# bwittmann/transoar

Measured on AMD Instinct MI355X. Metric: training-step CT volumes/s, 160x160x256 Focused-Decoder, higher is better.
Workload: dtype bf16

## Files before the change

include/transoar_convgemm.h:

```cpp
#ifndef TRANSOAR_CONVGEMM_H
#define TRANSOAR_CONVGEMM_H

#ifdef __cplusplus
extern "C" {
#endif

enum {
  TRANSOAR_CONVGEMM_OK = 0,
  TRANSOAR_CONVGEMM_ERR_NULL = -1,
  TRANSOAR_CONVGEMM_ERR_DIM = -2
};

int transoar_conv3d_igemm(const void* x, const void* wk, const float* bias, void* y, float* y32,
                          int N, int SD, int SH, int SW, int Cin, int Cout,
                          int MD, int MH, int MW, int src_stride,
                          int OD, int OH, int OW, int out_stride, int opd, int oph, int opw,
                          unsigned taps_d, unsigned taps_h, unsigned taps_w, int split, int classes, void* hip_stream);

int transoar_conv3d_finish(const float* y32, const float* bias, void* y, long rows, int cout, int split, void* hip_stream);

int transoar_conv3d_dgrad_s2_halo(const void* dy, const void* wkt, void* dx, int N, int OD, int OH, int OW, int D, int H, int W,
                                  int Cin, int Cout, void* hip_stream);

long transoar_conv3d_wgrad_part_floats(int Cin, int Cout, int chunks, int taps_out);
int transoar_conv3d_wgrad(const void* dy, const void* x, float* part, float* dw, int N, int SD, int SH, int SW, int Cin,
                          int Cout, int MD, int MH, int MW, int src_stride,
                          unsigned taps_d, unsigned taps_h, unsigned taps_w, int chunks, int taps_out, void* hip_stream);

int transoar_linear_wgrad_bias(const void* dy, const void* x, float* part, float* dw, float* bias_part, float* db, int T, int Cin,
                               int Cout, int chunks, void* hip_stream);

int transoar_conv3d_wgrad_ring(const void* dy, const void* x, float* part, float* dw, int N, int SD, int SH, int SW, int Cin,
                               int Cout, int MD, int MH, int MW, int src_stride, int chunks, void* hip_stream);

int transoar_conv3d_pack(const float* w, void* wk, void* wkt, int Cout, int Cin, void* hip_stream);

int transoar_conv3d_pack_many(const void* table, int n_layers, long total_tiles, void* hip_stream);

int transoar_convgemm_abi_version(void);

#ifdef __cplusplus
}
#endif
#endif
```

transoar_amd/conv_gemm.py:

```python
import ctypes
import os

import torch

from . import _native

_PKG = os.path.dirname(os.path.abspath(__file__))
_LIB_PATH = os.path.join(_PKG, "libtransoar_convgemm.so")
ABI_VERSION = 3
CL3D = torch.channels_last_3d


def _load():
    if not os.path.exists(_LIB_PATH):
        raise _native.NativeLibraryError("%s is not built (python transoar_amd/_build.py)" % _LIB_PATH)
    lib = ctypes.CDLL(_LIB_PATH)
    i, p, u = ctypes.c_int, ctypes.c_void_p, ctypes.c_uint
    lib.transoar_conv3d_igemm.restype = i
    lib.transoar_conv3d_igemm.argtypes = [p] * 5 + [i] * 17 + [u] * 3 + [i, i, p]
    lib.transoar_conv3d_finish.restype = i
    lib.transoar_conv3d_finish.argtypes = [p, p, p, ctypes.c_long, i, i, p]
    lib.transoar_conv3d_wgrad.restype = i
    lib.transoar_conv3d_wgrad.argtypes = [p, p, p, p] + [i] * 10 + [u] * 3 + [i, i, p]
    lib.transoar_linear_wgrad_bias.restype = i
    lib.transoar_linear_wgrad_bias.argtypes = [p] * 6 + [i] * 4 + [p]
    lib.transoar_conv3d_wgrad_ring.restype = i
    lib.transoar_conv3d_wgrad_ring.argtypes = [p, p, p, p] + [i] * 11 + [p]
    lib.transoar_conv3d_wgrad_part_floats.restype = ctypes.c_long
    lib.transoar_conv3d_wgrad_part_floats.argtypes = [i, i, i, i]
    lib.transoar_conv3d_dgrad_s2_halo.restype = i
    lib.transoar_conv3d_dgrad_s2_halo.argtypes = [p, p, p] + [i] * 9 + [p]
    lib.transoar_conv3d_pack.restype = i
    lib.transoar_conv3d_pack.argtypes = [p, p, p, i, i, p]
    lib.transoar_conv3d_pack_many.restype = i
    lib.transoar_conv3d_pack_many.argtypes = [p, i, ctypes.c_long, p]
    lib.transoar_convgemm_abi_version.restype = i
    if lib.transoar_convgemm_abi_version() != ABI_VERSION:
        raise _native.NativeLibraryError("%s: ABI mismatch, rebuild" % _LIB_PATH)
    return lib


lib = _load()


def _taps(entries):
    v = len(entries)
    for e, (delta, t) in enumerate(entries):
        v |= ((delta + 1) << (2 + 4 * e)) | (t << (4 + 4 * e))
    return v


TAPS_FWD = _taps([(-1, 0), (0, 1), (1, 2)])
TAPS_DGRAD1 = _taps([(1, 0), (0, 1), (-1, 2)])
TAPS_PARITY = (_taps([(0, 1)]), _taps([(1, 0), (0, 2)]))
TAPS_ONE = _taps([(0, 1)])

SPLIT_BELOW_TILES = 384
DGRAD_S2_HALO = os.environ.get("TRANSOAR_DGRAD_S2_HALO", "1") != "0"
WGRAD_BLOCKS = 512


def _check(rc, what):
    if rc != 0:
        raise RuntimeError("%s failed with code %d" % (what, rc))


def _stream():
    return torch.cuda.current_stream().cuda_stream


def pack_fwd(weight):
    co, ci = weight.shape[:2]
    return weight.permute(2, 3, 4, 0, 1).reshape(27, co, ci).to(torch.bfloat16).contiguous()


def pack_dgrad(weight):
    co, ci = weight.shape[:2]
    return weight.permute(2, 3, 4, 1, 0).reshape(27, ci, co).to(torch.bfloat16).contiguous()


def pack_both(weight):
    co, ci = weight.shape[:2]
    if weight.dtype != torch.float32 or not weight.is_contiguous() or not os.environ.get("TRANSOAR_CONV_PACK_HIP"):
        return pack_fwd(weight), pack_dgrad(weight)
    wk = torch.empty((27, co, ci), dtype=torch.bfloat16, device=weight.device)
    wkt = torch.empty((27, ci, co), dtype=torch.bfloat16, device=weight.device)
    with torch.cuda.device(weight.device):
        _check(lib.transoar_conv3d_pack(weight.data_ptr(), wk.data_ptr(), wkt.data_ptr(), co, ci, _stream()), "transoar_conv3d_pack")
    return wk, wkt


class PackPlan:

    def __init__(self, modules):
        self.modules = list(modules)
        assert self.modules
        dev = self.modules[0].weight.device
        self.buffers, rows, tile = [], [], 0
        for m in self.modules:
            w = m.weight
            assert w.dtype == torch.float32 and w.is_contiguous() and tuple(w.shape[2:]) == (3, 3, 3) and w.device == dev
            co, ci = w.shape[:2]
            wk = torch.empty((27, co, ci), dtype=torch.bfloat16, device=dev)
            wkt = torch.empty((27, ci, co), dtype=torch.bfloat16, device=dev)
            self.buffers.append((wk, wkt))
            rows.append([w.data_ptr(), wk.data_ptr(), wkt.data_ptr(), co | (ci << 32), tile])
            tile += ((co + 31) // 32) * ((ci + 31) // 32)
        self.total_tiles = tile
        self.ptrs = [r[0] for r in rows]
        self.table = torch.tensor(rows, dtype=torch.int64, device=dev)

    def valid(self):
        return all(m.weight.data_ptr() == p for m, p in zip(self.modules, self.ptrs))

    def run(self):
        with torch.cuda.device(self.table.device):
            _check(lib.transoar_conv3d_pack_many(self.table.data_ptr(), len(self.modules), self.total_tiles, _stream()),
                   "transoar_conv3d_pack_many")
        for m, packs in zip(self.modules, self.buffers):
            m._packs, m._packs_version = packs, m.weight._version


def _split_for(tiles, k_steps):
    if tiles >= SPLIT_BELOW_TILES:
        return 1
    return max(1, min((SPLIT_BELOW_TILES + tiles - 1) // tiles, k_steps // 4, 16))


def _tiles(rows, cout):
    bn = 64 if cout <= 64 else 128
    return ((rows + 127) // 128) * ((cout + bn - 1) // bn)


def _igemm(x, wk, bias, out, src_dims, cin, cout, m_dims, src_stride, out_dims, out_stride, parity, taps, n, split, classes=0):
    b = bias.data_ptr() if bias is not None else None
    with torch.cuda.device(x.device):
        if split > 1:
            rows_out = n * out_dims[0] * out_dims[1] * out_dims[2]
            part = torch.empty((split, rows_out, cout), dtype=torch.float32, device=x.device)
            _check(lib.transoar_conv3d_igemm(x.data_ptr(), wk.data_ptr(), None, None, part.data_ptr(), n, *src_dims, cin, cout,
                                             *m_dims, src_stride, *out_dims, out_stride, *parity, *taps, split, classes, _stream()),
                   "transoar_conv3d_igemm")
            _check(lib.transoar_conv3d_finish(part.data_ptr(), b, out.data_ptr(), rows_out, cout, split, _stream()),
                   "transoar_conv3d_finish")
        else:
            _check(lib.transoar_conv3d_igemm(x.data_ptr(), wk.data_ptr(), b, out.data_ptr(), None, n, *src_dims, cin, cout,
                                             *m_dims, src_stride, *out_dims, out_stride, *parity, *taps, 1, classes, _stream()),
                   "transoar_conv3d_igemm")


MAX_ROWS = 1 << 21


def _batch_chunks(n, rows_per_sample, what):
    if n * rows_per_sample < MAX_ROWS:
        return [(0, n)]
    per = (MAX_ROWS - 1) // rows_per_sample
    if per < 1:
        raise RuntimeError("%s: one sample has %d rows, the implicit-GEMM kernels address < %d per launch"
                           % (what, rows_per_sample, MAX_ROWS))
    return [(i, min(per, n - i)) for i in range(0, n, per)]


def conv_forward(x, wk, bias, stride, split=None):
    n, ci, d, h, w = x.shape
    co = wk.shape[1]
    od, oh, ow = (d - 1) // stride + 1, (h - 1) // stride + 1, (w - 1) // stride + 1
    chunks = _batch_chunks(n, od * oh * ow, "conv_forward")
    if len(chunks) > 1:
        y = torch.empty((n, co, od, oh, ow), dtype=torch.bfloat16, device=x.device, memory_format=CL3D)
        for i, c in chunks:
            y[i:i + c] = conv_forward(x[i:i + c], wk, bias, stride, split)
        return y
    y = torch.empty((n, co, od, oh, ow), dtype=torch.bfloat16, device=x.device, memory_format=CL3D)
    if split is None:
        split = _split_for(_tiles(n * od * oh * ow, co), (27 * ci + 63) // 64)
    _igemm(x, wk, bias, y, (d, h, w), ci, co, (od, oh, ow), stride, (od, oh, ow), 1, (0, 0, 0), (TAPS_FWD,) * 3, n, split)
    return y


def conv_dgrad(gy, wkt, stride, in_dims, split=None):
    n, co, od, oh, ow = gy.shape
    ci = wkt.shape[1]
    d, h, w = in_dims
    gx = torch.empty((n, ci, d, h, w), dtype=torch.bfloat16, device=gy.device, memory_format=CL3D)
    halo = split is None and stride == 2 and DGRAD_S2_HALO and ci <= 32 and co in (16, 32, 48)
    chunks = [(0, n)] if halo else _batch_chunks(n, d * h * w, "conv_dgrad")
    if len(chunks) > 1:
        for i, c in chunks:
            gx[i:i + c] = conv_dgrad(gy[i:i + c], wkt, stride, in_dims, split)
        return gx
    if stride == 1:
        if split is None:
            split = _split_for(_tiles(n * d * h * w, ci), (27 * co + 63) // 64)
        _igemm(gy, wkt, None, gx, (od, oh, ow), co, ci, (d, h, w), 1, (d, h, w), 1, (0, 0, 0), (TAPS_DGRAD1,) * 3, n, split)
        return gx
    if split is None and DGRAD_S2_HALO and ci <= 32 and co in (16, 32, 48):
        with torch.cuda.device(gy.device):
            _check(lib.transoar_conv3d_dgrad_s2_halo(gy.data_ptr(), wkt.data_ptr(), gx.data_ptr(), n, od, oh, ow, d, h, w, ci, co, _stream()),
                   "transoar_conv3d_dgrad_s2_halo")
        return gx
    if split is None:
        split = _split_for(_tiles(n * d * h * w, ci), (8 * co + 63) // 64)
    _igemm(gy, wkt, None, gx, (od, oh, ow), co, ci, (1, 1, 1), 1, (d, h, w), 2, (0, 0, 0), (TAPS_ONE,) * 3, n, split, classes=1)
    return gx


def _wgrad(x2, gy2, geom, taps, taps_out, out_shape):
    n, sd, sh, sw, ci, co, md, mh, mw, stride = geom
    nt = 1
    for t in taps:
        nt *= t & 3
    bt = 64 if (ci <= 64 and co <= 64) else 128
    tiles = nt * ((co + bt - 1) // bt) * ((ci + bt - 1) // bt)
    rows = n * md * mh * mw
    budget = WGRAD_BLOCKS * (2 if (rows >= (1 << 20) or tiles >= 64) else 1)
    chunks = max(1, min(budget // tiles, rows // 1024 if rows >= 1024 else 1))
    part = torch.empty(lib.transoar_conv3d_wgrad_part_floats(ci, co, chunks, taps_out), dtype=torch.float32, device=x2.device)
    dw = torch.empty(out_shape, dtype=torch.float32, device=x2.device)
    with torch.cuda.device(x2.device):
        _check(lib.transoar_conv3d_wgrad(gy2.data_ptr(), x2.data_ptr(), part.data_ptr(), dw.data_ptr(), n, sd, sh, sw, ci, co, md, mh, mw,
                                         stride, *taps, chunks, taps_out, _stream()), "transoar_conv3d_wgrad")
    return dw


WGRAD_RING = os.environ.get("TRANSOAR_WGRAD_RING", "1") != "0"
WGRAD_RING_CHUNKS = 85


def wgrad_ring_supported(ci, co, ow, rows):
    return (WGRAD_RING and ci <= 64 and co <= 64 and max(ci, co) > 32 and ci % 8 == 0 and co % 8 == 0 and ow % 64 == 0
            and rows >= (1 << 18))


def conv_wgrad_ring(x, gy, stride, chunks=None):
    n, ci, d, h, w = x.shape
    co, od, oh, ow = gy.shape[1:]
    chunks = chunks or WGRAD_RING_CHUNKS
    part = torch.empty(lib.transoar_conv3d_wgrad_part_floats(ci, co, chunks, 27), dtype=torch.float32, device=x.device)
    dw = torch.empty((co, ci, 3, 3, 3), dtype=torch.float32, device=x.device)
    with torch.cuda.device(x.device):
        _check(lib.transoar_conv3d_wgrad_ring(gy.data_ptr(), x.data_ptr(), part.data_ptr(), dw.data_ptr(), n, d, h, w, ci, co, od, oh, ow,
                                              stride, chunks, _stream()), "transoar_conv3d_wgrad_ring")
    return dw


def conv_wgrad(x, gy, stride):
    n, ci, d, h, w = x.shape
    co, od, oh, ow = gy.shape[1:]
    if wgrad_ring_supported(ci, co, ow, n * od * oh * ow):
        return conv_wgrad_ring(x, gy, stride)
    chunks = _batch_chunks(n, od * oh * ow, "conv_wgrad")
    if len(chunks) > 1:
        dw = None
        for i, c in chunks:
            part = conv_wgrad(x[i:i + c], gy[i:i + c], stride)
            dw = part if dw is None else dw.add_(part)
        return dw
    return _wgrad(x, gy, (n, d, h, w, ci, co, od, oh, ow, stride), (TAPS_FWD,) * 3, 27, (co, ci, 3, 3, 3))


def linear_wgrad(x, gy):
    t, k = x.shape
    nn_ = gy.shape[1]
    return _wgrad(x, gy, (1, 1, 1, t, k, nn_, 1, 1, t, 1), (TAPS_ONE,) * 3, 1, (nn_, k))


def linear_wgrad_bias_usable(k, n):
    return k % (64 if (k <= 64 and n <= 64) else 128) != 0


def linear_wgrad_bias(x, gy):
    t, k = x.shape
    nn_ = gy.shape[1]
    bt = 64 if (k <= 64 and nn_ <= 64) else 128
    tiles = ((nn_ + bt - 1) // bt) * ((k + bt - 1) // bt)
    budget = WGRAD_BLOCKS * (2 if (t >= (1 << 20) or tiles >= 64) else 1)
    chunks = max(1, min(budget // tiles, t // 1024 if t >= 1024 else 1))
    part = torch.empty(lib.transoar_conv3d_wgrad_part_floats(k, nn_, chunks, 1), dtype=torch.float32, device=x.device)
    bias_part = torch.empty(chunks * nn_, dtype=torch.float32, device=x.device)
    dw = torch.empty((nn_, k), dtype=torch.float32, device=x.device)
    db = torch.empty(nn_, dtype=torch.float32, device=x.device)
    with torch.cuda.device(x.device):
        _check(lib.transoar_linear_wgrad_bias(gy.data_ptr(), x.data_ptr(), part.data_ptr(), dw.data_ptr(), bias_part.data_ptr(), db.data_ptr(),
                                              t, k, nn_, chunks, _stream()), "transoar_linear_wgrad_bias")
    return dw, db


def supported(cin, cout, rows):
    return cin % 8 == 0 and cout % 8 == 0 and cin >= 8 and rows < (1 << 21)
```

transoar_amd/csrc/conv_gemm.hip:

```cpp
#include <hip/hip_runtime.h>
#include <stdint.h>

#include "../../include/transoar_convgemm.h"

namespace {

typedef float f32x16 __attribute__((ext_vector_type(16)));
typedef short s16x8 __attribute__((ext_vector_type(8)));
typedef short s16x4 __attribute__((ext_vector_type(4)));
typedef __bf16 bf16x8_t __attribute__((ext_vector_type(8)));
typedef unsigned int u32x4 __attribute__((ext_vector_type(4)));

constexpr int BM = 128, BK = 64;
constexpr int kTile = BM * BK * 2;

__device__ __forceinline__ f32x16 mfma(s16x8 a, s16x8 b, f32x16 c) {
  return __builtin_amdgcn_mfma_f32_32x32x16_bf16(__builtin_bit_cast(bf16x8_t, a), __builtin_bit_cast(bf16x8_t, b), c, 0, 0, 0);
}
__device__ __forceinline__ unsigned short f32_to_bf16(float f) {
  return __builtin_bit_cast(unsigned short, static_cast<__bf16>(f));
}
typedef __attribute__((address_space(3))) void conv_lds_void;
__device__ __forceinline__ void dma16(__amdgpu_buffer_rsrc_t rs, unsigned voff, unsigned dst) {
  unsigned keep;
// ... 278 lines not shown
    for (int e = 0; e < 8; ++e) v[e] += bias[c + e];
  }
  u32x4 o;
#pragma unroll
  for (int e = 0; e < 4; ++e) o[e] = static_cast<unsigned>(f32_to_bf16(v[2 * e])) | (static_cast<unsigned>(f32_to_bf16(v[2 * e + 1])) << 16);
  reinterpret_cast<u32x4*>(y)[i] = o;
}

constexpr int WK = 64;
constexpr int kSegRows = 2048;

template <int TW>
__global__ __launch_bounds__(256, 2) void conv3d_wgrad_kernel(
    const unsigned short* __restrict__ DY, const unsigned short* __restrict__ X, float* __restrict__ part, ConvGeom g,
    unsigned tp_d, unsigned tp_h, unsigned tp_w, int chunks, int rows_per_chunk, int tiles_co, int tiles_ci, int slabs,
    unsigned dy_bytes, unsigned x_bytes, float* __restrict__ bias_part) {
  constexpr int BT = 64 * TW;
  constexpr int WP = 2 * BT;
  constexpr int PR = 8 * TW;
  __shared__ __attribute__((aligned(16))) unsigned char lds[2][2 * WK * WP];
  __shared__ unsigned xrow[kSegRows];
  const int tid = threadIdx.x, lane = tid & 63, wave = tid >> 6;
  const int wm = wave >> 1, wn = wave & 1;
  const int nd = taps_count(tp_d), nh = taps_count(tp_h), nw = taps_count(tp_w);
  const int ntaps = nd * nh * nw;
  long bid = xcd_contiguous(blockIdx.x, static_cast<long>(chunks) * tiles_ci * tiles_co * ntaps);
  if (bid < 0) return;
  const int tci = static_cast<int>(bid % tiles_ci); bid /= tiles_ci;
  const int tco = static_cast<int>(bid % tiles_co); bid /= tiles_co;
  const int tap = static_cast<int>(bid % ntaps); bid /= ntaps;
  const int chunk = static_cast<int>(bid);
  const int ed = tap / (nh * nw), r_ = tap - ed * nh * nw, eh = r_ / nw, ew = r_ - eh * nw;
  const int dd = taps_delta(tp_d, ed), dh = taps_delta(tp_h, eh), dw = taps_delta(tp_w, ew);
  const int slab = (taps_t(tp_d, ed) * 3 + taps_t(tp_h, eh)) * 3 + taps_t(tp_w, ew);
  const int M = g.N * g.MD * g.MH * g.MW;
  const int m_beg = chunk * rows_per_chunk, m_end = min(M, m_beg + rows_per_chunk);
  const int co0 = tco * BT, ci0 = tci * BT;
  const __amdgpu_buffer_rsrc_t rdy = __builtin_amdgcn_make_buffer_rsrc(const_cast<unsigned short*>(DY), 0, static_cast<int>(dy_bytes), 0x00020000);
  const __amdgpu_buffer_rsrc_t rx = __builtin_amdgcn_make_buffer_rsrc(const_cast<unsigned short*>(X), 0, static_cast<int>(x_bytes), 0x00020000);

  constexpr int NS = WK * PR / 256, RS = 256 / PR;
  const int s_piece = tid % PR, s_row = tid / PR;
  auto row_swz = [](int r) -> int { return TW == 2 ? (r & 3) << 2 : ((r >> 1) & 1) << 2; };
  const int l_piece = s_piece ^ row_swz(s_row);
  const bool co_ok = co0 + l_piece * 8 < g.Cout, ci_ok = ci0 + l_piece * 8 < g.Cin;
  const unsigned y_col = co_ok ? static_cast<unsigned>(co0 + l_piece * 8) * 2u : 0x80000000u;
  const unsigned x_col = ci_ok ? static_cast<unsigned>(ci0 + l_piece * 8) * 2u : 0x80000000u;
  const bool bias_here = bias_part != nullptr && tci == tiles_ci - 1;
  const bool ones_piece = bias_here && ci0 + l_piece * 8 == g.Cin;
  if (ones_piece) {
#pragma unroll
    for (int st = 0; st < 2; ++st)
#pragma unroll
      for (int i = 0; i < WK * PR / 256; ++i)
        *reinterpret_cast<u32x4*>(&lds[st][WK * WP + (s_row + (256 / PR) * i) * WP + s_piece * 16]) = u32x4{0x00003f80u, 0u, 0u, 0u};
  }
  const float inv_mw = 1.0f / static_cast<float>(g.MW), inv_mh = 1.0f / static_cast<float>(g.MH), inv_md = 1.0f / static_cast<float>(g.MD);
  auto fill_rows = [&](int seg_beg, int seg_end) {
    for (int m = seg_beg + tid; m < seg_end; m += 256) {
      const int r1 = static_cast<int>((static_cast<float>(m) + 0.5f) * inv_mw), mw = m - r1 * g.MW;
      const int r2 = static_cast<int>((static_cast<float>(r1) + 0.5f) * inv_mh), mh = r1 - r2 * g.MH;
      const int nb = static_cast<int>((static_cast<float>(r2) + 0.5f) * inv_md), md = r2 - nb * g.MD;
      const int sd = md * g.src_stride + dd, sh = mh * g.src_stride + dh, sw = mw * g.src_stride + dw;
      const bool ok = static_cast<unsigned>(sd) < static_cast<unsigned>(g.SD) && static_cast<unsigned>(sh) < static_cast<unsigned>(g.SH) &&
                      static_cast<unsigned>(sw) < static_cast<unsigned>(g.SW);
      xrow[m - seg_beg] = ok ? static_cast<unsigned>(((nb * g.SD + sd) * g.SH + sh) * g.SW + sw) * static_cast<unsigned>(g.Cin) * 2u : 0x80000000u;
    }
  };
  int seg0 = 0, seg1 = 0;
  const unsigned lds0 = static_cast<unsigned>(reinterpret_cast<size_t>((conv_lds_void*)&lds[0][0]));
  const unsigned dst0 = __builtin_amdgcn_readfirstlane(lds0 + static_cast<unsigned>(wave) * 1024u);
  auto dma_step = [&](int m_base, int stage) {
    const unsigned base = dst0 + static_cast<unsigned>(stage) * (2u * WK * WP);
#pragma unroll
    for (int i = 0; i < NS; ++i) {
      const int m = m_base + s_row + RS * i;
      const bool in = m < seg1;
      const unsigned xo = in ? xrow[m - seg0] : 0x80000000u;
      dma16(rdy, in ? static_cast<unsigned>(m) * static_cast<unsigned>(g.Cout) * 2u + y_col : 0x80000000u, base + i * (RS * WP));
      if (!ones_piece) dma16(rx, xo + x_col, base + WK * WP + i * (RS * WP));
    }
  };
  f32x16 acc[TW][TW];
#pragma unroll
  for (int a = 0; a < TW; ++a)
#pragma unroll
    for (int b = 0; b < TW; ++b)
#pragma unroll
      for (int i = 0; i < 16; ++i) acc[a][b][i] = 0.f;
  const int kg = lane >> 5;
  const int t_row = 8 * kg + ((lane & 15) >> 2), t_ch = 16 * ((lane >> 4) & 1) + 4 * (lane & 3);
  typedef __attribute__((address_space(3))) s16x4 lds_s16x4;
  const int t_swz = row_swz(t_row) * 16;
  auto frag = [&](const unsigned char* tile, int k16, int ch0) -> s16x8 {
    const unsigned char* p = tile + (k16 * 16 + t_row) * WP + (((ch0 + t_ch) * 2) ^ t_swz);
    const s16x4 lo = __builtin_amdgcn_ds_read_tr16_b64_v4i16((lds_s16x4*)(p));
    const s16x4 hi = __builtin_amdgcn_ds_read_tr16_b64_v4i16((lds_s16x4*)(p + 4 * WP));
    return __builtin_shufflevector(lo, hi, 0, 1, 2, 3, 4, 5, 6, 7);
  };
  auto compute = [&](int stage) {
    const unsigned char* ty = lds[stage];
    const unsigned char* tx = lds[stage] + WK * WP;
#pragma unroll
    for (int k16 = 0; k16 < WK / 16; ++k16) {
      s16x8 fy[TW], fx[TW];
#pragma unroll
      for (int i = 0; i < TW; ++i) {
        fy[i] = frag(ty, k16, wm * 32 * TW + i * 32);
        fx[i] = frag(tx, k16, wn * 32 * TW + i * 32);
      }
#pragma unroll
      for (int a = 0; a < TW; ++a)
#pragma unroll
        for (int b = 0; b < TW; ++b) acc[a][b] = mfma(fy[a], fx[b], acc[a][b]);
    }
  };
  for (seg0 = m_beg; seg0 < m_end; seg0 += kSegRows) {
    seg1 = min(m_end, seg0 + kSegRows);
    __syncthreads();
    fill_rows(seg0, seg1);
    __syncthreads();
    const int steps = (seg1 - seg0 + WK - 1) / WK;
    dma_step(seg0, 0);
    dma_wait();
    block_barrier();
    for (int s = 0; s < steps; s += 2) {
      if (s + 1 < steps) dma_step(seg0 + (s + 1) * WK, 1);
      compute(0);
      dma_wait();
      block_barrier();
      if (s + 1 >= steps) break;
      if (s + 2 < steps) dma_step(seg0 + (s + 2) * WK, 0);
      compute(1);
      dma_wait();
      block_barrier();
    }
  }
  float* dst = part + (static_cast<long>(chunk) * slabs + (slabs == 1 ? 0 : slab)) * g.Cout * g.Cin;
#pragma unroll
  for (int a = 0; a < TW; ++a)
#pragma unroll
    for (int b = 0; b < TW; ++b) {
      const int ci = ci0 + wn * 32 * TW + b * 32 + (lane & 31);
      if (bias_here && ci == g.Cin) {
#pragma unroll
        for (int r = 0; r < 16; ++r) {
          const int co = co0 + wm * 32 * TW + a * 32 + (r & 3) + 8 * (r >> 2) + 4 * kg;
          if (co < g.Cout) bias_part[static_cast<long>(chunk) * g.Cout + co] = acc[a][b][r];
        }
      }
      if (ci >= g.Cin) continue;
#pragma unroll
      for (int r = 0; r < 16; ++r) {
        const int co = co0 + wm * 32 * TW + a * 32 + (r & 3) + 8 * (r >> 2) + 4 * kg;
        if (co < g.Cout) dst[static_cast<long>(co) * g.Cin + ci] = acc[a][b][r];
      }
    }
}

constexpr int kReducePairs = 128;
__global__ __launch_bounds__(256) void conv3d_wgrad_reduce_kernel(const float* __restrict__ part, float* __restrict__ dw, int chunks,
                                                                  int slabs, long coci) {
  __shared__ __attribute__((aligned(16))) float sh[kReducePairs * 27];
  const long e0 = static_cast<long>(blockIdx.x) * kReducePairs;
  const int quads = kReducePairs / 4;
  const int work = quads * slabs;
  if (work < 256) {
    const int P = 256 / work;
    const int sub = threadIdx.x / work, idx = threadIdx.x - sub * work;
    const int tap = idx / quads, q = idx - tap * quads;
    float4 v{0.f, 0.f, 0.f, 0.f};
    if (sub < P && e0 + 4 * q < coci) {
      const float* src = part + static_cast<long>(tap) * coci + e0 + 4 * q;
      const long step = static_cast<long>(slabs) * coci;
      int k = sub;
      for (; k + 3 * P < chunks; k += 4 * P) {
        const float4 a = *reinterpret_cast<const float4*>(src + (k + 0 * P) * step), b = *reinterpret_cast<const float4*>(src + (k + 1 * P) * step);
        const float4 c = *reinterpret_cast<const float4*>(src + (k + 2 * P) * step), d = *reinterpret_cast<const float4*>(src + (k + 3 * P) * step);
        v.x += (a.x + b.x) + (c.x + d.x); v.y += (a.y + b.y) + (c.y + d.y);
        v.z += (a.z + b.z) + (c.z + d.z); v.w += (a.w + b.w) + (c.w + d.w);
      }
      for (; k < chunks; k += P) {
        const float4 a = *reinterpret_cast<const float4*>(src + k * step);
        v.x += a.x; v.y += a.y; v.z += a.z; v.w += a.w;
      }
    }
    float4* turn = reinterpret_cast<float4*>(sh);
    if (sub < P) turn[sub * work + idx] = v;
    __syncthreads();
    if (sub == 0) {
      for (int g2 = 1; g2 < P; ++g2) {
        const float4 o = turn[g2 * work + idx];
        v.x += o.x; v.y += o.y; v.z += o.z; v.w += o.w;
      }
    }
    __syncthreads();
    if (sub == 0) {
      sh[(4 * q + 0) * slabs + tap] = v.x;
      sh[(4 * q + 1) * slabs + tap] = v.y;
      sh[(4 * q + 2) * slabs + tap] = v.z;
      sh[(4 * q + 3) * slabs + tap] = v.w;
    }
  } else {
  for (int idx = threadIdx.x; idx < quads * slabs; idx += 256) {
    const int tap = idx / quads, q = idx - tap * quads;
    float4 v{0.f, 0.f, 0.f, 0.f};
    if (e0 + 4 * q < coci) {
      const float* src = part + static_cast<long>(tap) * coci + e0 + 4 * q;
      const long step = static_cast<long>(slabs) * coci;
      int k = 0;
      for (; k + 4 <= chunks; k += 4) {
        const float4 a = *reinterpret_cast<const float4*>(src + (k + 0) * step), b = *reinterpret_cast<const float4*>(src + (k + 1) * step);
        const float4 c = *reinterpret_cast<const float4*>(src + (k + 2) * step), d = *reinterpret_cast<const float4*>(src + (k + 3) * step);
        v.x += (a.x + b.x) + (c.x + d.x); v.y += (a.y + b.y) + (c.y + d.y);
        v.z += (a.z + b.z) + (c.z + d.z); v.w += (a.w + b.w) + (c.w + d.w);
      }
      for (; k < chunks; ++k) {
        const float4 a = *reinterpret_cast<const float4*>(src + k * step);
        v.x += a.x; v.y += a.y; v.z += a.z; v.w += a.w;
      }
    }
    sh[(4 * q + 0) * slabs + tap] = v.x;
    sh[(4 * q + 1) * slabs + tap] = v.y;
    sh[(4 * q + 2) * slabs + tap] = v.z;
    sh[(4 * q + 3) * slabs + tap] = v.w;
  }
  }
  __syncthreads();
  const long total = coci * slabs, base = e0 * slabs;
  for (int idx = threadIdx.x; idx < quads * slabs; idx += 256)
    if (base + 4 * idx < total) *reinterpret_cast<float4*>(dw + base + 4 * idx) = *reinterpret_cast<const float4*>(&sh[4 * idx]);
}

__global__ __launch_bounds__(256) void conv3d_pack_kernel(const float* __restrict__ w, unsigned short* __restrict__ wk,
                                                          unsigned short* __restrict__ wkt, int co_n, int ci_n) {
  __shared__ unsigned short sh[27][32][33];
  const int tiles_ci = (ci_n + 31) / 32;
  const int co0 = (blockIdx.x / tiles_ci) * 32, ci0 = (blockIdx.x % tiles_ci) * 32;
  for (int idx = threadIdx.x; idx < 32 * 32 * 27; idx += 256) {
    const int col = idx % (32 * 27), a = idx / (32 * 27);
    const int b = col / 27, tap = col - b * 27;
    const int co = co0 + a, ci = ci0 + b;
    float v = 0.f;
    if (co < co_n && ci < ci_n) v = w[(static_cast<long>(co) * ci_n + ci) * 27 + tap];
    sh[tap][a][b] = f32_to_bf16(v);
  }
  __syncthreads();
  for (int idx = threadIdx.x; idx < 27 * 32 * 32; idx += 256) {
    const int x = idx & 31, y = (idx >> 5) & 31, tap = idx >> 10;
    if (co0 + y < co_n && ci0 + x < ci_n) wk[(static_cast<long>(tap) * co_n + co0 + y) * ci_n + ci0 + x] = sh[tap][y][x];
    if (wkt != nullptr && ci0 + y < ci_n && co0 + x < co_n) wkt[(static_cast<long>(tap) * ci_n + ci0 + y) * co_n + co0 + x] = sh[tap][x][y];
  }
}

struct PackEntry {
  const float* w;
  unsigned short* wk;
  unsigned short* wkt;
  long co_ci;
  long tile_begin;
};
__global__ __launch_bounds__(256) void conv3d_pack_many_kernel(const PackEntry* __restrict__ table, int n_layers) {
  constexpr int P = 34;
  __shared__ __attribute__((aligned(16))) unsigned short sh[27][32][P];
  int l = 0;
  while (l + 1 < n_layers && static_cast<long>(blockIdx.x) >= table[l + 1].tile_begin) ++l;
  const PackEntry e = table[l];
  const int co_n = static_cast<int>(e.co_ci & 0xffffffffL), ci_n = static_cast<int>(e.co_ci >> 32);
  const int tile = static_cast<int>(blockIdx.x - e.tile_begin);
  const int tiles_ci = (ci_n + 31) / 32;
  const int co0 = (tile / tiles_ci) * 32, ci0 = (tile % tiles_ci) * 32;
  const int ci_valid = min(32, ci_n - ci0);
  for (int idx = threadIdx.x; idx < 32 * 216; idx += 256) {
    const int a = idx / 216, f = idx - a * 216;
    float4 v{0.f, 0.f, 0.f, 0.f};
    if (co0 + a < co_n && 4 * f < ci_valid * 27)
      v = *reinterpret_cast<const float4*>(e.w + (static_cast<long>(co0 + a) * ci_n + ci0) * 27 + 4 * f);
    const float vv[4] = {v.x, v.y, v.z, v.w};
#pragma unroll
    for (int j = 0; j < 4; ++j) {
      const int p = 4 * f + j, b = p / 27, tap = p - b * 27;
      sh[tap][a][b] = f32_to_bf16(vv[j]);
    }
  }
  __syncthreads();
  for (int idx = threadIdx.x; idx < 27 * 32 * 4; idx += 256) {
    const int x8 = idx & 3, y = (idx >> 2) & 31, tap = idx >> 7;
    if (co0 + y < co_n && ci0 + 8 * x8 < ci_n) {
      const unsigned* src = reinterpret_cast<const unsigned*>(&sh[tap][y][8 * x8]);
      *reinterpret_cast<u32x4*>(e.wk + (static_cast<long>(tap) * co_n + co0 + y) * ci_n + ci0 + 8 * x8) = u32x4{src[0], src[1], src[2], src[3]};
    }
    if (e.wkt != nullptr && ci0 + y < ci_n && co0 + 8 * x8 < co_n) {
      unsigned r[4];
#pragma unroll
      for (int j = 0; j < 4; ++j)
        r[j] = static_cast<unsigned>(sh[tap][8 * x8 + 2 * j][y]) | (static_cast<unsigned>(sh[tap][8 * x8 + 2 * j + 1][y]) << 16);
      *reinterpret_cast<u32x4*>(e.wkt + (static_cast<long>(tap) * ci_n + ci0 + y) * co_n + co0 + 8 * x8) = u32x4{r[0], r[1], r[2], r[3]};
    }
  }
}

#include "conv_dgrad_s2.hpp"
#include "conv_wgrad_ring.hpp"

int check_geom(const ConvGeom& g) {
  if (g.N <= 0 || g.SD <= 0 || g.SH <= 0 || g.SW <= 0 || g.MD <= 0 || g.MH <= 0 || g.MW <= 0 || g.OD <= 0 || g.OH <= 0 || g.OW <= 0 ||
      g.Cin <= 0 || g.Cout <= 0 || (g.Cin & 7) || (g.Cout & 7) || g.src_stride < 1 || g.src_stride > 2 || g.out_stride < 1 || g.out_stride > 2)
    return TRANSOAR_CONVGEMM_ERR_DIM;
  const long src = static_cast<long>(g.N) * g.SD * g.SH * g.SW * g.Cin * 2, out = static_cast<long>(g.N) * g.OD * g.OH * g.OW * g.Cout * 2;
  const long rows = static_cast<long>(g.N) * g.MD * g.MH * g.MW;
  if (src >= 0x7ffffff0L || out >= 0x7ffffff0L * 2 || rows >= (1L << 31) || rows * g.Cout * 2 >= 0x7ffffff0L * 2 || 27L * g.Cout * g.Cin * 2 >= 0x3ffffff0L)
    return TRANSOAR_CONVGEMM_ERR_DIM;
  return 0;
}
bool taps_ok(unsigned p) { return (p & 3) >= 1 && (p & 3) <= 3; }

}

extern "C" int transoar_conv3d_igemm(const void* x, const void* wk, const float* bias, void* y, float* y32, int N, int SD,
                                     int SH, int SW, int Cin, int Cout, int MD, int MH, int MW, int src_stride, int OD, int OH,
                                     int OW, int out_stride, int opd, int oph, int opw, unsigned taps_d, unsigned taps_h,
                                     unsigned taps_w, int split, int classes, void* hip_stream) {
  if (!x || !wk || (!y && !y32)) return TRANSOAR_CONVGEMM_ERR_NULL;
  if (classes) {
    MD = (OD + 1) / 2; MH = (OH + 1) / 2; MW = (OW + 1) / 2;
    src_stride = 1; out_stride = 2; opd = oph = opw = 0;
    taps_d = taps_h = taps_w = kTapsParity1;
  }
  const ConvGeom g{N, SD, SH, SW, MD, MH, MW, OD, OH, OW, src_stride, out_stride, opd, oph, opw, Cin, Cout};
  const int rc = check_geom(g);
  if (rc) return rc;
  if (!taps_ok(taps_d) || !taps_ok(taps_h) || !taps_ok(taps_w) || split < 1 || (split > 1 && !y32)) return TRANSOAR_CONVGEMM_ERR_DIM;
  if (static_cast<long>(N) * MD * MH * MW >= (1L << 21)) return TRANSOAR_CONVGEMM_ERR_DIM;
  hipStream_t st = static_cast<hipStream_t>(hip_stream);
  const bool narrow = Cout <= 64;
  const int bn = narrow ? 64 : 128;
  const int tiles_n = (Cout + bn - 1) / bn;
  long n_tiles = 0;
  if (classes) {
    for (int c = 0; c < 8; ++c) {
      const long md = (OD - ((c >> 2) & 1) + 1) / 2, mh = (OH - ((c >> 1) & 1) + 1) / 2, mw = (OW - (c & 1) + 1) / 2;
      n_tiles += (N * md * mh * mw + BM - 1) / BM * tiles_n;
    }
  } else {
    n_tiles = (static_cast<long>(N) * MD * MH * MW + BM - 1) / BM * tiles_n;
  }
  const long blocks = ((n_tiles * split + 7) / 8) * 8;
  const unsigned xb = static_cast<unsigned>(static_cast<long>(N) * SD * SH * SW * Cin * 2), wb = static_cast<unsigned>(27L * Cout * Cin * 2);
  if (narrow)
    hipLaunchKernelGGL(conv3d_igemm_kernel<1>, dim3(static_cast<unsigned>(blocks)), dim3(256), 0, st, static_cast<const unsigned short*>(x),
                       static_cast<const unsigned short*>(wk), bias, static_cast<unsigned short*>(y), y32, g, taps_d, taps_h, taps_w,
                       split, n_tiles, tiles_n, classes, xb, wb);
  else
    hipLaunchKernelGGL(conv3d_igemm_kernel<2>, dim3(static_cast<unsigned>(blocks)), dim3(256), 0, st, static_cast<const unsigned short*>(x),
                       static_cast<const unsigned short*>(wk), bias, static_cast<unsigned short*>(y), y32, g, taps_d, taps_h, taps_w,
                       split, n_tiles, tiles_n, classes, xb, wb);
  return static_cast<int>(hipGetLastError());
}

extern "C" int transoar_conv3d_dgrad_s2_halo(const void* dy, const void* wkt, void* dx, int N, int OD, int OH, int OW, int D, int H, int W,
                                            int Cin, int Cout, void* hip_stream) {
  if (!dy || !wkt || !dx) return TRANSOAR_CONVGEMM_ERR_NULL;
  if (N <= 0 || OD <= 0 || OH <= 0 || OW <= 0 || Cin <= 0 || Cin > 32 || (Cin & 7) || (Cout != 16 && Cout != 32 && Cout != 48))
    return TRANSOAR_CONVGEMM_ERR_DIM;
  if ((D != 2 * OD && D != 2 * OD - 1) || (H != 2 * OH && H != 2 * OH - 1) || (W != 2 * OW && W != 2 * OW - 1)) return TRANSOAR_CONVGEMM_ERR_DIM;
  const long dy_bytes = static_cast<long>(N) * OD * OH * OW * Cout * 2;
  if (dy_bytes >= 0x7ffffff0L || (4L * H + 8) * W * Cin * 2 >= 0x7ffffff0L) return TRANSOAR_CONVGEMM_ERR_DIM;
  const int td = (OD + kDs2TD - 1) / kDs2TD, th = (OH + kDs2TH - 1) / kDs2TH, tw = (OW + kDs2TW - 1) / kDs2TW;
  const long n_tiles = static_cast<long>(N) * td * th * tw;
  static int resident[3] = {0, 0, 0};
  const int ki = Cout / 16 - 1;
  if (!resident[ki]) {
    int per_cu = 0, dev = 0;
    hipDeviceProp_t prop;
    const void* fn = ki == 0 ? reinterpret_cast<const void*>(conv3d_dgrad_s2_halo_kernel<1>)
                   : ki == 1 ? reinterpret_cast<const void*>(conv3d_dgrad_s2_halo_kernel<2>) : reinterpret_cast<const void*>(conv3d_dgrad_s2_halo_kernel<3>);
    if (hipGetDevice(&dev) != hipSuccess || hipGetDeviceProperties(&prop, dev) != hipSuccess ||
        hipOccupancyMaxActiveBlocksPerMultiprocessor(&per_cu, fn, 256, 0) != hipSuccess || per_cu < 1)
      return TRANSOAR_CONVGEMM_ERR_DIM;
    resident[ki] = per_cu * prop.multiProcessorCount;
  }
  const unsigned blocks = static_cast<unsigned>(n_tiles < resident[ki] ? n_tiles : resident[ki]);
  hipStream_t st = static_cast<hipStream_t>(hip_stream);
#define TRANSOAR_DS2_LAUNCH(KS)                                                                                                     \
  hipLaunchKernelGGL(conv3d_dgrad_s2_halo_kernel<KS>, dim3(blocks), dim3(256), 0, st, static_cast<const unsigned short*>(dy),       \
                     static_cast<const unsigned short*>(wkt), static_cast<unsigned short*>(dx), N, OD, OH, OW, D, H, W, Cin, td, th, tw, \
                     static_cast<unsigned>(dy_bytes))
  if (Cout == 16) TRANSOAR_DS2_LAUNCH(1);
  else if (Cout == 32) TRANSOAR_DS2_LAUNCH(2);
  else TRANSOAR_DS2_LAUNCH(3);
#undef TRANSOAR_DS2_LAUNCH
  return static_cast<int>(hipGetLastError());
}

extern "C" int transoar_conv3d_finish(const float* y32, const float* bias, void* y, long rows, int cout, int split, void* hip_stream) {
  if (!y32 || !y) return TRANSOAR_CONVGEMM_ERR_NULL;
  if (rows <= 0 || cout <= 0 || (cout & 7) || split < 1) return TRANSOAR_CONVGEMM_ERR_DIM;
  const long n8 = rows * cout / 8;
  hipLaunchKernelGGL(conv3d_finish_kernel, dim3(static_cast<unsigned>((n8 + 255) / 256)), dim3(256), 0, static_cast<hipStream_t>(hip_stream),
                     y32, bias, static_cast<unsigned short*>(y), n8, cout, split);
  return static_cast<int>(hipGetLastError());
}

extern "C" long transoar_conv3d_wgrad_part_floats(int Cin, int Cout, int chunks, int taps_out) { return static_cast<long>(taps_out) * Cin * Cout * chunks; }

static int wgrad_launch(const void* dy, const void* x, float* part, float* dw, int N, int SD, int SH, int SW, int Cin,
                        int Cout, int MD, int MH, int MW, int src_stride, unsigned taps_d, unsigned taps_h,
                        unsigned taps_w, int chunks, int taps_out, float* bias_part, float* db, void* hip_stream) {
  if (!dy || !x || !part || !dw) return TRANSOAR_CONVGEMM_ERR_NULL;
  const ConvGeom g{N, SD, SH, SW, MD, MH, MW, MD, MH, MW, src_stride, 1, 0, 0, 0, Cin, Cout};
  const int rc = check_geom(g);
  if (rc) return rc;
  if (!taps_ok(taps_d) || !taps_ok(taps_h) || !taps_ok(taps_w) || chunks < 1 || (taps_out != 1 && taps_out != 27)) return TRANSOAR_CONVGEMM_ERR_DIM;
  const long M = static_cast<long>(N) * MD * MH * MW;
  if (M >= (1L << 21)) return TRANSOAR_CONVGEMM_ERR_DIM;
  const int max_chunks = chunks;
  if (chunks > M) chunks = static_cast<int>(M);
  const int rows_per_chunk = static_cast<int>(((M + chunks - 1) / chunks + WK - 1) / WK * WK);
  chunks = static_cast<int>((M + rows_per_chunk - 1) / rows_per_chunk);
  if (chunks > max_chunks) return TRANSOAR_CONVGEMM_ERR_DIM;
  const int ntaps = static_cast<int>((taps_d & 3) * (taps_h & 3) * (taps_w & 3));
  if (taps_out == 1 && ntaps != 1) return TRANSOAR_CONVGEMM_ERR_DIM;
  hipStream_t st = static_cast<hipStream_t>(hip_stream);
  const bool small = Cin <= 64 && Cout <= 64;
  const int bt = small ? 64 : 128;
  const int tiles_co = (Cout + bt - 1) / bt, tiles_ci = (Cin + bt - 1) / bt;
  const long blocks = (static_cast<long>(chunks) * tiles_ci * tiles_co * ntaps + 7) / 8 * 8;
  if (blocks >= (1L << 31)) return TRANSOAR_CONVGEMM_ERR_DIM;
  const unsigned dyb = static_cast<unsigned>(M * Cout * 2), xb = static_cast<unsigned>(static_cast<long>(N) * SD * SH * SW * Cin * 2);
  if (small)
    hipLaunchKernelGGL(conv3d_wgrad_kernel<1>, dim3(static_cast<unsigned>(blocks)), dim3(256), 0, st, static_cast<const unsigned short*>(dy),
                       static_cast<const unsigned short*>(x), part, g, taps_d, taps_h, taps_w, chunks, rows_per_chunk, tiles_co, tiles_ci, taps_out, dyb, xb, bias_part);
  else
    hipLaunchKernelGGL(conv3d_wgrad_kernel<2>, dim3(static_cast<unsigned>(blocks)), dim3(256), 0, st, static_cast<const unsigned short*>(dy),
                       static_cast<const unsigned short*>(x), part, g, taps_d, taps_h, taps_w, chunks, rows_per_chunk, tiles_co, tiles_ci, taps_out, dyb, xb, bias_part);
  const long coci = static_cast<long>(Cout) * Cin;
  hipLaunchKernelGGL(conv3d_wgrad_reduce_kernel, dim3(static_cast<unsigned>((coci + kReducePairs - 1) / kReducePairs)), dim3(256), 0, st, part, dw, chunks, taps_out, coci);
  if (bias_part != nullptr)
    hipLaunchKernelGGL(conv3d_wgrad_reduce_kernel, dim3(static_cast<unsigned>((Cout + kReducePairs - 1) / kReducePairs)), dim3(256), 0, st, bias_part, db, chunks, 1,
                       static_cast<long>(Cout));
  return static_cast<int>(hipGetLastError());
}

extern "C" int transoar_conv3d_wgrad(const void* dy, const void* x, float* part, float* dw, int N, int SD, int SH, int SW, int Cin,
                                     int Cout, int MD, int MH, int MW, int src_stride, unsigned taps_d, unsigned taps_h,
                                     unsigned taps_w, int chunks, int taps_out, void* hip_stream) {
  return wgrad_launch(dy, x, part, dw, N, SD, SH, SW, Cin, Cout, MD, MH, MW, src_stride, taps_d, taps_h, taps_w, chunks, taps_out, nullptr, nullptr,
                      hip_stream);
}

extern "C" int transoar_linear_wgrad_bias(const void* dy, const void* x, float* part, float* dw, float* bias_part, float* db, int T,
                                          int Cin, int Cout, int chunks, void* hip_stream) {
  if (!bias_part || !db) return TRANSOAR_CONVGEMM_ERR_NULL;
  const int bt = (Cin <= 64 && Cout <= 64) ? 64 : 128;
  if (Cin % bt == 0) return TRANSOAR_CONVGEMM_ERR_DIM;
  constexpr unsigned kOneTap = 1u | (1u << 2) | (1u << 4);
  return wgrad_launch(dy, x, part, dw, 1, 1, 1, T, Cin, Cout, 1, 1, T, 1, kOneTap, kOneTap, kOneTap, chunks, 1, bias_part, db, hip_stream);
}

extern "C" int transoar_conv3d_wgrad_ring(const void* dy, const void* x, float* part, float* dw, int N, int SD, int SH, int SW, int Cin,
                                          int Cout, int MD, int MH, int MW, int src_stride, int chunks, void* hip_stream) {
  if (!dy || !x || !part || !dw) return TRANSOAR_CONVGEMM_ERR_NULL;
  if (N <= 0 || SD <= 0 || SH <= 0 || SW <= 0 || MD <= 0 || MH <= 0 || MW <= 0 || Cin <= 0 || Cout <= 0 || (Cin & 7) || (Cout & 7) ||
      Cin > 64 || Cout > 64 || (MW & 63) || chunks < 1 || (src_stride != 1 && src_stride != 2))
    return TRANSOAR_CONVGEMM_ERR_DIM;
  if (MD != (SD - 1) / src_stride + 1 || MH != (SH - 1) / src_stride + 1 || MW != (SW - 1) / src_stride + 1) return TRANSOAR_CONVGEMM_ERR_DIM;
  const int tiles_co = (Cout + 31) / 32, tiles_ci = (Cin + 31) / 32;
  if (tiles_co * tiles_ci < 2) return TRANSOAR_CONVGEMM_ERR_DIM;
  const long columns = static_cast<long>(N) * MD * (MW / 64);
  int h_chunks = 1;
  while (columns * h_chunks < 4L * chunks && (MH + h_chunks) / (h_chunks + 1) >= 8) ++h_chunks;
  const int h_chunk = (MH + h_chunks - 1) / h_chunks;
  h_chunks = (MH + h_chunk - 1) / h_chunk;
  hipStream_t st = static_cast<hipStream_t>(hip_stream);
  const dim3 grid(static_cast<unsigned>(chunks * 3));
  auto dys = static_cast<const unsigned short*>(dy);
  auto xs = static_cast<const unsigned short*>(x);
#define TRANSOAR_RING_LAUNCH(S_, CIT_)                                                                                                    \
  hipLaunchKernelGGL((conv3d_wgrad_ring_kernel<S_, CIT_>), grid, dim3(512), 0, st, dys, xs, part, N, SD, SH, SW, MD, MH, MW, Cin, Cout, tiles_co, \
                     tiles_ci, h_chunks, h_chunk)
  if (src_stride == 1) { if (tiles_ci == 1) TRANSOAR_RING_LAUNCH(1, 1); else TRANSOAR_RING_LAUNCH(1, 2); }
  else { if (tiles_ci == 1) TRANSOAR_RING_LAUNCH(2, 1); else TRANSOAR_RING_LAUNCH(2, 2); }
#undef TRANSOAR_RING_LAUNCH
  const long coci = static_cast<long>(Cout) * Cin;
  hipLaunchKernelGGL(conv3d_wgrad_reduce_kernel, dim3(static_cast<unsigned>((coci + kReducePairs - 1) / kReducePairs)), dim3(256), 0, st, part, dw, chunks, 27, coci);
  return static_cast<int>(hipGetLastError());
}

extern "C" int transoar_conv3d_pack(const float* w, void* wk, void* wkt, int Cout, int Cin, void* hip_stream) {
  if (!w || !wk) return TRANSOAR_CONVGEMM_ERR_NULL;
  if (Cout <= 0 || Cin <= 0) return TRANSOAR_CONVGEMM_ERR_DIM;
  const int blocks = ((Cout + 31) / 32) * ((Cin + 31) / 32);
  hipLaunchKernelGGL(conv3d_pack_kernel, dim3(blocks), dim3(256), 0, static_cast<hipStream_t>(hip_stream), w,
                     static_cast<unsigned short*>(wk), static_cast<unsigned short*>(wkt), Cout, Cin);
  return static_cast<int>(hipGetLastError());
}

extern "C" int transoar_conv3d_pack_many(const void* table, int n_layers, long total_tiles, void* hip_stream) {
  if (!table) return TRANSOAR_CONVGEMM_ERR_NULL;
  if (n_layers <= 0 || total_tiles <= 0 || total_tiles >= (1L << 31)) return TRANSOAR_CONVGEMM_ERR_DIM;
  hipLaunchKernelGGL(conv3d_pack_many_kernel, dim3(static_cast<unsigned>(total_tiles)), dim3(256), 0, static_cast<hipStream_t>(hip_stream),
                     static_cast<const PackEntry*>(table), n_layers);
  return static_cast<int>(hipGetLastError());
}

extern "C" int transoar_convgemm_abi_version(void) { return 3; }
```

Baseline: 63.99.

## Add kw-reuse wgrad kernel sharing one dy tile across three width taps

Adds a new weight-gradient kernel for stride-1 3x3x3 convs with wide channels (>64). Each block handles one (kd,kh) tap pair and computes all three kw taps from a single loaded dy tile and a slightly wider x tile with a halo, which cuts global loads and LDS traffic compared with the generic per-tap path. Partial sums per chunk are written out and reduced by the existing reduce kernel. The change adds a row-offset table, float-based index division and a new dispatch path that is on by default through an environment flag.

```diff
diff --git a/include/transoar_convgemm.h b/include/transoar_convgemm.h
--- a/include/transoar_convgemm.h
+++ b/include/transoar_convgemm.h
@@ -33,6 +33,9 @@
 int transoar_conv3d_wgrad_ring(const void* dy, const void* x, float* part, float* dw, int N, int SD, int SH, int SW, int Cin,
                                int Cout, int MD, int MH, int MW, int src_stride, int chunks, void* hip_stream);
 
+int transoar_conv3d_wgrad_kw3(const void* dy, const void* x, float* part, float* dw, int N, int D, int H, int W, int Cin,
+                              int Cout, int chunks, void* hip_stream);
+
 int transoar_conv3d_pack(const float* w, void* wk, void* wkt, int Cout, int Cin, void* hip_stream);
 
 int transoar_conv3d_pack_many(const void* table, int n_layers, long total_tiles, void* hip_stream);
diff --git a/transoar_amd/conv_gemm.py b/transoar_amd/conv_gemm.py
--- a/transoar_amd/conv_gemm.py
+++ b/transoar_amd/conv_gemm.py
@@ -7,7 +7,7 @@
 
 _PKG = os.path.dirname(os.path.abspath(__file__))
 _LIB_PATH = os.path.join(_PKG, "libtransoar_convgemm.so")
-ABI_VERSION = 3
+ABI_VERSION = 4
 CL3D = torch.channels_last_3d
 
 
@@ -26,6 +26,8 @@
     lib.transoar_linear_wgrad_bias.argtypes = [p] * 6 + [i] * 4 + [p]
     lib.transoar_conv3d_wgrad_ring.restype = i
     lib.transoar_conv3d_wgrad_ring.argtypes = [p, p, p, p] + [i] * 11 + [p]
+    lib.transoar_conv3d_wgrad_kw3.restype = i
+    lib.transoar_conv3d_wgrad_kw3.argtypes = [p, p, p, p] + [i] * 7 + [p]
     lib.transoar_conv3d_wgrad_part_floats.restype = ctypes.c_long
     lib.transoar_conv3d_wgrad_part_floats.argtypes = [i, i, i, i]
     lib.transoar_conv3d_dgrad_s2_halo.restype = i
@@ -245,16 +247,44 @@
     return dw
 
 
-def conv_wgrad(x, gy, stride):
+WGRAD_KW3 = os.environ.get("TRANSOAR_WGRAD_KW3", "1") != "0"
+WGRAD_KW3_MIN_ROWS = 512
+WGRAD_KW3_BLOCKS = 512
+
+
+def wgrad_kw3_supported(ci, co, w, stride):
+    return WGRAD_KW3 and stride == 1 and max(ci, co) > 64 and ci % 8 == 0 and co % 8 == 0 and w % 4 == 0
+
+
+def conv_wgrad_kw3(x, gy, chunks=None):
+    n, ci, d, h, w = x.shape
+    co = gy.shape[1]
+    rows = n * d * h * w
+    if chunks is None:
+        tiles = 9 * ((co + 127) // 128) * ((ci + 63) // 64)
+        chunks = max(1, min(WGRAD_KW3_BLOCKS // tiles, rows // 512))
+        if rows // chunks > 16384:
+            chunks = max(1, 2 * WGRAD_KW3_BLOCKS // tiles)
+    part = torch.empty(lib.transoar_conv3d_wgrad_part_floats(ci, co, chunks, 27), dtype=torch.float32, device=x.device)
+    dw = torch.empty((co, ci, 3, 3, 3), dtype=torch.float32, device=x.device)
+    with torch.cuda.device(x.device):
+        _check(lib.transoar_conv3d_wgrad_kw3(gy.data_ptr(), x.data_ptr(), part.data_ptr(), dw.data_ptr(), n, d, h, w, ci, co, chunks,
+                                             _stream()), "transoar_conv3d_wgrad_kw3")
+    return dw
+
+
+def conv_wgrad(x, gy, stride, _kw3=True):
     n, ci, d, h, w = x.shape
     co, od, oh, ow = gy.shape[1:]
     if wgrad_ring_supported(ci, co, ow, n * od * oh * ow):
         return conv_wgrad_ring(x, gy, stride)
+    if _kw3 and wgrad_kw3_supported(ci, co, w, stride) and WGRAD_KW3_MIN_ROWS <= n * od * oh * ow < MAX_ROWS:
+        return conv_wgrad_kw3(x, gy)
     chunks = _batch_chunks(n, od * oh * ow, "conv_wgrad")
     if len(chunks) > 1:
         dw = None
         for i, c in chunks:
-            part = conv_wgrad(x[i:i + c], gy[i:i + c], stride)
+            part = conv_wgrad(x[i:i + c], gy[i:i + c], stride, _kw3=False)
             dw = part if dw is None else dw.add_(part)
         return dw
     return _wgrad(x, gy, (n, d, h, w, ci, co, od, oh, ow, stride), (TAPS_FWD,) * 3, 27, (co, ci, 3, 3, 3))
diff --git a/transoar_amd/csrc/conv_gemm.hip b/transoar_amd/csrc/conv_gemm.hip
--- a/transoar_amd/csrc/conv_gemm.hip
+++ b/transoar_amd/csrc/conv_gemm.hip
@@ -604,6 +604,7 @@
 
 #include "conv_dgrad_s2.hpp"
 #include "conv_wgrad_ring.hpp"
+#include "conv_wgrad_kw.hpp"
 
 int check_geom(const ConvGeom& g) {
   if (g.N <= 0 || g.SD <= 0 || g.SH <= 0 || g.SW <= 0 || g.MD <= 0 || g.MH <= 0 || g.MW <= 0 || g.OD <= 0 || g.OH <= 0 || g.OW <= 0 ||
@@ -789,6 +790,32 @@
   return static_cast<int>(hipGetLastError());
 }
 
+extern "C" int transoar_conv3d_wgrad_kw3(const void* dy, const void* x, float* part, float* dw, int N, int D, int H, int W, int Cin,
+                                         int Cout, int chunks, void* hip_stream) {
+  if (!dy || !x || !part || !dw) return TRANSOAR_CONVGEMM_ERR_NULL;
+  const ConvGeom g{N, D, H, W, D, H, W, D, H, W, 1, 1, 0, 0, 0, Cin, Cout};
+  const int rc = check_geom(g);
+  if (rc) return rc;
+  if ((W & 3) || chunks < 1) return TRANSOAR_CONVGEMM_ERR_DIM;
+  const long M = static_cast<long>(N) * D * H * W;
+  if (M >= (1L << 21)) return TRANSOAR_CONVGEMM_ERR_DIM;
+  const int max_chunks = chunks;
+  if (chunks > M) chunks = static_cast<int>(M);
+  const int rows_per_chunk = static_cast<int>(((M + chunks - 1) / chunks + WK - 1) / WK * WK);
+  chunks = static_cast<int>((M + rows_per_chunk - 1) / rows_per_chunk);
+  if (chunks > max_chunks) return TRANSOAR_CONVGEMM_ERR_DIM;
+  const int tiles_co = (Cout + kKwCo - 1) / kKwCo, tiles_ci = (Cin + kKwCi - 1) / kKwCi;
+  const long blocks = (static_cast<long>(chunks) * tiles_ci * tiles_co * 9 + 7) / 8 * 8;
+  if (blocks >= (1L << 31)) return TRANSOAR_CONVGEMM_ERR_DIM;
+  hipStream_t st = static_cast<hipStream_t>(hip_stream);
+  hipLaunchKernelGGL(conv3d_wgrad_kw3_kernel, dim3(static_cast<unsigned>(blocks)), dim3(256), 0, st, static_cast<const unsigned short*>(dy),
+                     static_cast<const unsigned short*>(x), part, N, D, H, W, Cin, Cout, chunks, rows_per_chunk, tiles_co, tiles_ci,
+                     static_cast<unsigned>(M * Cout * 2), static_cast<unsigned>(M * Cin * 2));
+  const long coci = static_cast<long>(Cout) * Cin;
+  hipLaunchKernelGGL(conv3d_wgrad_reduce_kernel, dim3(static_cast<unsigned>((coci + kReducePairs - 1) / kReducePairs)), dim3(256), 0, st, part, dw, chunks, 27, coci);
+  return static_cast<int>(hipGetLastError());
+}
+
 extern "C" int transoar_conv3d_pack(const float* w, void* wk, void* wkt, int Cout, int Cin, void* hip_stream) {
   if (!w || !wk) return TRANSOAR_CONVGEMM_ERR_NULL;
   if (Cout <= 0 || Cin <= 0) return TRANSOAR_CONVGEMM_ERR_DIM;
@@ -806,4 +833,4 @@
   return static_cast<int>(hipGetLastError());
 }
 
-extern "C" int transoar_convgemm_abi_version(void) { return 3; }
+extern "C" int transoar_convgemm_abi_version(void) { return 4; }
diff --git a/transoar_amd/csrc/conv_wgrad_kw.hpp b/transoar_amd/csrc/conv_wgrad_kw.hpp
--- /dev/null
+++ b/transoar_amd/csrc/conv_wgrad_kw.hpp
@@ -0,0 +1,179 @@
+#pragma once
+
+constexpr int kKwCo = 128, kKwCi = 64;
+constexpr int kKwDyTile = WK * kKwCo * 2;
+constexpr int kKwXRows = 96;
+constexpr int kKwXTile = kKwXRows * kKwCi * 2;
+
+__global__ __launch_bounds__(256, 2) void conv3d_wgrad_kw3_kernel(
+    const unsigned short* __restrict__ DY, const unsigned short* __restrict__ X, float* __restrict__ part, int N, int D, int H, int W,
+    int Cin, int Cout, int chunks, int rows_per_chunk, int tiles_co, int tiles_ci, unsigned dy_bytes, unsigned x_bytes) {
+  constexpr int WPY = kKwCo * 2, WPX = kKwCi * 2;
+  constexpr unsigned kStage = kKwDyTile + kKwXTile;
+  __shared__ __attribute__((aligned(16))) unsigned char lds[2][kStage];
+  __shared__ unsigned xrow[kSegRows + 2];
+  const int tid = threadIdx.x, lane = tid & 63, wave = tid >> 6;
+  const int wm = wave >> 1, wn = wave & 1;
+  long bid = xcd_contiguous(blockIdx.x, static_cast<long>(chunks) * tiles_ci * tiles_co * 9);
+  if (bid < 0) return;
+  const int tci = static_cast<int>(bid % tiles_ci); bid /= tiles_ci;
+  const int tco = static_cast<int>(bid % tiles_co); bid /= tiles_co;
+  const int khd = static_cast<int>(bid % 9); bid /= 9;
+  const int chunk = static_cast<int>(bid);
+  const int kd = khd / 3, kh = khd - 3 * kd;
+  const int dd = kd - 1, dh = kh - 1;
+  const int M = N * D * H * W;
+  const int m_beg = chunk * rows_per_chunk, m_end = min(M, m_beg + rows_per_chunk);
+  const int co0 = tco * kKwCo, ci0 = tci * kKwCi;
+  const __amdgpu_buffer_rsrc_t rdy = __builtin_amdgcn_make_buffer_rsrc(const_cast<unsigned short*>(DY), 0, static_cast<int>(dy_bytes), 0x00020000);
+  const __amdgpu_buffer_rsrc_t rx = __builtin_amdgcn_make_buffer_rsrc(const_cast<unsigned short*>(X), 0, static_cast<int>(x_bytes), 0x00020000);
+
+  const int y_row = tid >> 4, y_piece = (tid & 15) ^ ((y_row & 3) << 2);
+  const unsigned y_col = co0 + y_piece * 8 < Cout ? static_cast<unsigned>(co0 + y_piece * 8) * 2u : 0x80000000u;
+  const int x_row = wave * 8 + (lane >> 3), x_piece = (lane & 7) ^ (((x_row >> 1) & 1) << 2);
+  const unsigned x_col = ci0 + x_piece * 8 < Cin ? static_cast<unsigned>(ci0 + x_piece * 8) * 2u : 0x80000000u;
+
+  const float inv_w = 1.0f / static_cast<float>(W), inv_h = 1.0f / static_cast<float>(H), inv_d = 1.0f / static_cast<float>(D);
+  auto fill_rows = [&](int seg_beg, int seg_end) {
+    for (int m = seg_beg - 1 + tid; m <= seg_end; m += 256) {
+      unsigned v = 0x80000000u;
+      if (m >= 0 && m < M) {
+        const int r1 = static_cast<int>((static_cast<float>(m) + 0.5f) * inv_w), mw = m - r1 * W;
+        const int r2 = static_cast<int>((static_cast<float>(r1) + 0.5f) * inv_h), mh = r1 - r2 * H;
+        const int nb = static_cast<int>((static_cast<float>(r2) + 0.5f) * inv_d), md = r2 - nb * D;
+        const int sd = md + dd, sh = mh + dh;
+        if (static_cast<unsigned>(sd) < static_cast<unsigned>(D) && static_cast<unsigned>(sh) < static_cast<unsigned>(H))
+          v = static_cast<unsigned>(((nb * D + sd) * H + sh) * W + mw) * static_cast<unsigned>(Cin) * 2u;
+      }
+      xrow[m - (seg_beg - 1)] = v;
+    }
+  };
+  int seg0 = 0, seg1 = 0;
+
+  const float inv_w1 = 1.0f / static_cast<float>(W + 1);
+  const int kg = lane >> 5;
+  const int t_row = 8 * kg + ((lane & 15) >> 2), t_ch = 16 * ((lane >> 4) & 1) + 4 * (lane & 3);
+  int x_j[3];
+  int x_rows = 0;
+  int fx_off[4][2][3];
+  constexpr int kNoVoxel = -64;
+  auto layout_dma = [&](int w0) {
+#pragma unroll
+    for (int i = 0; i < 3; ++i) {
+      const int e = w0 - 1 + x_row + 32 * i;
+      int j = kNoVoxel;
+      if (e >= 0) {
+        const int q = static_cast<int>((static_cast<float>(e) + 0.5f) * inv_w1), s = e - q * (W + 1);
+        if (s < W) j = q * W + s - w0;
+      }
+      x_j[i] = j <= 64 ? j : kNoVoxel;
+    }
+    x_rows = __builtin_amdgcn_readfirstlane(66 + static_cast<int>((static_cast<float>(w0 + 63) + 0.5f) * inv_w));
+  };
+  auto layout_read = [&](int w0) {
+#pragma unroll
+    for (int k16 = 0; k16 < 4; ++k16)
+#pragma unroll
+      for (int hf = 0; hf < 2; ++hf) {
+        const int j = k16 * 16 + t_row + 4 * hf;
+        const int r1 = 1 + j + static_cast<int>((static_cast<float>(w0 + j) + 0.5f) * inv_w);
+#pragma unroll
+        for (int kw = 0; kw < 3; ++kw) {
+          const int r = r1 + kw - 1;
+          fx_off[k16][hf][kw] = r * WPX + (((wn * 32 + t_ch) * 2) ^ (((r >> 1) & 1) << 6));
+        }
+      }
+  };
+  const bool w_fixed = (64 % W) == 0;
+  layout_dma(0);
+  layout_read(0);
+
+  const unsigned lds0 = static_cast<unsigned>(reinterpret_cast<size_t>((conv_lds_void*)&lds[0][0]));
+  const unsigned dst0 = __builtin_amdgcn_readfirstlane(lds0 + static_cast<unsigned>(wave) * 1024u);
+  auto dma_step = [&](int m_base, int stage) {
+    const unsigned base = dst0 + static_cast<unsigned>(stage) * kStage;
+    if (!w_fixed) layout_dma(m_base % W);
+#pragma unroll
+    for (int i = 0; i < 4; ++i) {
+      const int m = m_base + y_row + 16 * i;
+      dma16(rdy, m < seg1 ? static_cast<unsigned>(m) * static_cast<unsigned>(Cout) * 2u + y_col : 0x80000000u, base + i * 4096u);
+    }
+#pragma unroll
+    for (int i = 0; i < 3; ++i) {
+      if ((4 * i + wave) * 8 >= x_rows) break;
+      const int m = m_base + x_j[i];
+      const unsigned xo = (x_j[i] != kNoVoxel && m <= seg1) ? xrow[m - (seg0 - 1)] : 0x80000000u;
+      dma16(rx, xo + x_col, base + kKwDyTile + i * 4096u);
+    }
+  };
+
+  f32x16 acc[3][2];
+#pragma unroll
+  for (int t = 0; t < 3; ++t)
+#pragma unroll
+    for (int a = 0; a < 2; ++a)
+#pragma unroll
+      for (int i = 0; i < 16; ++i) acc[t][a][i] = 0.f;
+  typedef __attribute__((address_space(3))) s16x4 lds_s16x4;
+  const int fy_off = t_row * WPY + (((wm * 64 + t_ch) * 2) ^ ((t_row & 3) << 6));
+  auto tr8 = [&](const unsigned char* lo, const unsigned char* hi) -> s16x8 {
+    const s16x4 a = __builtin_amdgcn_ds_read_tr16_b64_v4i16((lds_s16x4*)(lo));
+    const s16x4 b = __builtin_amdgcn_ds_read_tr16_b64_v4i16((lds_s16x4*)(hi));
+    return __builtin_shufflevector(a, b, 0, 1, 2, 3, 4, 5, 6, 7);
+  };
+  auto compute = [&](int stage, int m_base) {
+    if (!w_fixed) layout_read(m_base % W);
+    const unsigned char* ty = lds[stage];
+    const unsigned char* tx = lds[stage] + kKwDyTile;
+#pragma unroll
+    for (int k16 = 0; k16 < 4; ++k16) {
+      s16x8 fy[2], fx[3];
+#pragma unroll
+      for (int a = 0; a < 2; ++a) {
+        const unsigned char* p = ty + k16 * 16 * WPY + (fy_off ^ (a << 6));
+        fy[a] = tr8(p, p + 4 * WPY);
+      }
+#pragma unroll
+      for (int kw = 0; kw < 3; ++kw) fx[kw] = tr8(tx + fx_off[k16][0][kw], tx + fx_off[k16][1][kw]);
+#pragma unroll
+      for (int kw = 0; kw < 3; ++kw)
+#pragma unroll
+        for (int a = 0; a < 2; ++a) acc[kw][a] = mfma(fy[a], fx[kw], acc[kw][a]);
+    }
+  };
+  for (seg0 = m_beg; seg0 < m_end; seg0 += kSegRows) {
+    seg1 = min(m_end, seg0 + kSegRows);
+    __syncthreads();
+    fill_rows(seg0, seg1);
+    __syncthreads();
+    const int steps = (seg1 - seg0 + WK - 1) / WK;
+    dma_step(seg0, 0);
+    dma_wait();
+    block_barrier();
+    for (int s = 0; s < steps; s += 2) {
+      if (s + 1 < steps) dma_step(seg0 + (s + 1) * WK, 1);
+      compute(0, seg0 + s * WK);
+      dma_wait();
+      block_barrier();
+      if (s + 1 >= steps) break;
+      if (s + 2 < steps) dma_step(seg0 + (s + 2) * WK, 0);
+      compute(1, seg0 + (s + 1) * WK);
+      dma_wait();
+      block_barrier();
+    }
+  }
+  const int ci = ci0 + wn * 32 + (lane & 31);
+  if (ci >= Cin) return;
+  const long coci = static_cast<long>(Cout) * Cin;
+#pragma unroll
+  for (int kw = 0; kw < 3; ++kw) {
+    float* dst = part + (static_cast<long>(chunk) * 27 + khd * 3 + kw) * coci;
+#pragma unroll
+    for (int a = 0; a < 2; ++a)
+#pragma unroll
+      for (int r = 0; r < 16; ++r) {
+        const int co = co0 + wm * 64 + a * 32 + (r & 3) + 8 * (r >> 2) + 4 * kg;
+        if (co < Cout) dst[static_cast<long>(co) * Cin + ci] = acc[kw][a][r];
+      }
+  }
+}
```

New measurement: 63.96. About the same (-0.0%).
